# lucieDLE/TMRNet

Hardware: AMD Instinct MI355X
Metric: train frames/sec, TMRNet ResNet50 seq=10 LFB=40 (higher is better)
Workload: dtype fp32; 1 GPU; C2/C3: TMRNet ResNet50+LSTM+NLBlock train step; model=resnet_lstm (train_only_non-local_pretrained), global_batch=64, clips_per_gpu=64, seq_len=10, lfb_len=40, parallelism=dp1, input_transform=reference train transform (use_flip=1) on device

## Files before the change

### include/tmr.h

```cpp
#ifndef TMR_H_
#define TMR_H_

#ifdef TMR_HOST_ONLY
typedef struct ihipStream_t* hipStream_t;
#else
#include <hip/hip_runtime.h>
#endif
#include <stddef.h>
#include <stdint.h>

#ifdef __cplusplus
extern "C" {
#endif

#define TMR_ABI_VERSION 8

int tmr_abi_version(void);
const char* tmr_last_error(void);
void tmr_clear_error(void);

typedef struct tmr_conv_desc {
  int n, h, w, c;
  int k;
  int r, s, stride, pad;
// ... 347 lines not shown
                    void* ws, size_t ws_bytes, hipStream_t stream);


int tmr_linear_fwd(const float* x, int rows, int in, int out, const float* w, const float* bias,
                   float* y, hipStream_t stream);
int tmr_linear_bwd(const float* dy, const float* x, int rows, int in, int out, const float* w,
                   float* dx, float* dw, float* db, float beta, hipStream_t stream);

typedef struct tmr_nlblock_weights {
  const float *w1, *b1, *w2, *b2, *w3, *b3, *ln_w, *ln_b, *w4, *b4;
} tmr_nlblock_weights;
typedef struct tmr_nlblock_grads {
  float *w1, *b1, *w2, *b2, *w3, *b3, *ln_w, *ln_b, *w4, *b4;
} tmr_nlblock_grads;
size_t tmr_nlblock_saved_bytes(int b, int l);
size_t tmr_nlblock_ws_bytes(int b, int l);
int tmr_nlblock_fwd(const tmr_nlblock_weights* w, const float* st, const float* lt,
                    const int32_t* rows, int b, int l, const float* mask, float* out, void* saved,
                    size_t saved_bytes, void* ws, size_t ws_bytes, hipStream_t stream);
int tmr_nlblock_bwd(const tmr_nlblock_weights* w, const float* dout, const float* st,
                    const float* lt, const int32_t* rows, int b, int l, const float* mask,
                    const void* saved, size_t saved_bytes, float* dst, float* dlt,
                    const tmr_nlblock_grads* g, void* ws, size_t ws_bytes, hipStream_t stream);

size_t tmr_timeconv_saved_bytes(int b, int l);
size_t tmr_timeconv_ws_bytes(int b, int l);
int tmr_timeconv_fwd(const float* x, int b, int l, const float* w3, const float* b3,
                     const float* w5, const float* b5, const float* w7, const float* b7,
                     float* out, void* saved, size_t saved_bytes, void* ws, size_t ws_bytes,
                     hipStream_t stream);
int tmr_timeconv_wgrad(const float* dy, const float* x, int b, int l, const float* w3,
                       const float* w5, const float* w7, const void* saved, size_t saved_bytes,
                       float* dx, float* dw3, float* db3, float* dw5, float* db5, float* dw7,
                       float* db7, void* ws, size_t ws_bytes, hipStream_t stream);

size_t tmr_lstm_saved_bytes(int b, int t, int h);
size_t tmr_lstm_ws_bytes(int b, int t, int i, int h);
int tmr_lstm_fwd(const float* x, int b, int t, int i, int h, const float* w_ih,
                 const float* w_hh, const float* b_ih, const float* b_hh, float* y, float* hn,
                 float* cn, void* saved, size_t saved_bytes, void* ws, size_t ws_bytes,
                 hipStream_t stream);
int tmr_lstm_bwd(const float* dy, const float* x, int b, int t, int i, int h, const float* w_ih,
                 const float* w_hh, const float* y, const void* saved, size_t saved_bytes,
                 float* dx, float* dw_ih, float* dw_hh, float* db_ih, float* db_hh, void* ws,
                 size_t ws_bytes, hipStream_t stream);
size_t tmr_lstm_window_ws_bytes(int b, int t, int h);
int tmr_lstm_window_fwd(const float* gates, long nrows, const int32_t* rows, int b, int t, int h,
                        const float* w_hh, float* out, const int32_t* out_rows, void* ws,
                        size_t ws_bytes, hipStream_t stream);
int tmr_lstm_sync_status(const void* ws, unsigned* timeout_out, hipStream_t stream);
int tmr_lstm_status_or(const void* ws, int32_t* status, hipStream_t stream);
int tmr_test_hold_cus(int wgs, float ms, hipStream_t stream);
long tmr_dgrad_ws_launches(void);

int tmr_timeconv_max5_fwd(const float* x, const float* y1, const float* y2, const float* y3,
                          float* out, uint8_t* code, int b, int l, int c, hipStream_t stream);
int tmr_timeconv_max5_bwd(const float* dy, const uint8_t* code, float* d1, float* d2, float* d3,
                          float* dx, int b, int l, int c, hipStream_t stream);

int tmr_lstm_cell_fwd(const float* gx, int ldgx, const float* ghh, const float* c_prev,
                      float* h_out, int ldh, float* c_out, float* act, int b, int hdim,
                      hipStream_t stream);
int tmr_lstm_cell_bwd(const float* dh_out, int lddh, const float* dh_rec, const float* dc_next,
                      const float* act, const float* c, const float* c_prev, float* dgates,
                      int lddg, float* dc_prev, int b, int hdim, hipStream_t stream);

#ifdef __cplusplus
}
#endif
#endif
```

### tmrnet_amd/_lib.py

```python
import ctypes
import os

import torch

_HERE = os.path.dirname(os.path.abspath(__file__))
LIB_PATH = os.environ.get("TMR_LIB_PATH") or os.path.join(_HERE, "libtmr.so")

P = ctypes.c_void_p
I = ctypes.c_int
L = ctypes.c_long
F = ctypes.c_float
U64 = ctypes.c_uint64
SZ = ctypes.c_size_t


class ConvDesc(ctypes.Structure):
    _fields_ = [(n, ctypes.c_int) for n in
                ("n", "h", "w", "c", "k", "r", "s", "stride", "pad", "ho", "wo", "pad_w",
                 "x_ld", "y_ld", "math", "max_frames", "io", "groups")]


DP = ctypes.POINTER(ConvDesc)


# ... 100 lines not shown
    "tmr_splat_gap_bn": [P, P, P, P, I, I, I, I, P],
    "tmr_splat_att": [P, P, I, I, P],
    "tmr_splat_combine_bn": [P, P, P, P, P, I, I, I, I, P],
    "tmr_splat_bwd_reduce_bn": [P, P, P, P, P, P, P, P, I, I, I, I, P],
    "tmr_splat_bn0_coefs": [P, P, P, P, P, P, P, P, P, I, I, I, P],
    "tmr_splat_bwd_apply_bn": [P, P, P, P, P, P, P, P, P, I, I, I, I, P],
    "tmr_avgpool2d_fwd_a16": [P, P, I, I, I, I, I, I, I, I, I, I, P],
    "tmr_fill_f32": [P, L, F, P],
    "tmr_seq_last": [P, P, I, I, I, P],
    "tmr_seq_last_bwd": [P, P, P, I, I, I, P],
    "tmr_counters_add": [P, I, ctypes.c_int64, P],
    "tmr_center_cols": [P, I, I, P, P, P],
    "tmr_axpy": [I, F, P, P, P],
    "tmr_avgpool2d_fwd": [P, P, I, I, I, I, I, I, I, I, I, I, P],
    "tmr_avgpool2d_bwd": [P, P, I, I, I, I, I, I, I, I, I, I, P],
    "tmr_col_sum": [P, I, I, I, P, F, P],
    "tmr_dropout_mask": [P, L, F, U64, U64, P],
    "tmr_softmax_max": [P, I, I, P, P, P, P],
    "tmr_ce_sum": [P, P, P, I, I, F, P, P, P, P],
    "tmr_sgd_chunk": [],
    "tmr_sgd_step_multi": [P, I, ctypes.c_int64, P, P],
    "tmr_sgd_step": [P, P, P, L, F, F, F, F, I, I, P],
    "tmr_lfb_index": [P, I, P, I, I, P, P],
    "tmr_lfb_gather": [P, P, P, L, I, P],
    "tmr_layernorm_relu_fwd": [P, P, P, P, P, P, I, I, F, P],
    "tmr_layernorm_relu_bwd": [P, P, P, P, P, P, P, P, P, I, I, P],
    "tmr_residual_mask": [P, P, P, P, L, P],
    "tmr_mask_relu_fwd": [P, P, P, L, P],
    "tmr_mask_relu_bwd": [P, P, P, P, L, P],
    "tmr_mul": [P, P, P, P, L, P],
    "tmr_nl_attn_ws_bytes": [I, I, I],
    "tmr_nl_attn_fwd": [P, P, P, P, P, I, I, I, F, P, SZ, P],
    "tmr_nl_attn_bwd": [P, P, P, P, P, P, P, I, I, I, F, P, SZ, P],
    "tmr_linear_fwd": [P, I, I, I, P, P, P, P],
    "tmr_linear_bwd": [P, P, I, I, I, P, P, P, P, F, P],
    "tmr_nlblock_saved_bytes": [I, I],
    "tmr_nlblock_ws_bytes": [I, I],
    "tmr_nlblock_fwd": [P, P, P, P, I, I, P, P, P, SZ, P, SZ, P],
    "tmr_nlblock_bwd": [P, P, P, P, P, I, I, P, P, SZ, P, P, P, P, SZ, P],
    "tmr_timeconv_saved_bytes": [I, I],
    "tmr_timeconv_ws_bytes": [I, I],
    "tmr_timeconv_fwd": [P, I, I, P, P, P, P, P, P, P, P, SZ, P, SZ, P],
    "tmr_timeconv_wgrad": [P, P, I, I, P, P, P, P, SZ, P, P, P, P, P, P, P, P, SZ, P],
    "tmr_lstm_saved_bytes": [I, I, I],
    "tmr_lstm_ws_bytes": [I, I, I, I],
    "tmr_lstm_fwd": [P, I, I, I, I, P, P, P, P, P, P, P, P, SZ, P, SZ, P],
    "tmr_lstm_bwd": [P, P, I, I, I, I, P, P, P, P, SZ, P, P, P, P, P, P, SZ, P],
    "tmr_lstm_window_ws_bytes": [I, I, I],
    "tmr_lstm_window_fwd": [P, L, P, I, I, I, P, P, P, P, SZ, P],
    "tmr_lstm_sync_status": [P,ctypes.POINTER(ctypes.c_uint), P],
    "tmr_lstm_status_or": [P, P, P],
    "tmr_test_hold_cus": [I, F, P],
    "tmr_dgrad_ws_launches": [],
    "tmr_timeconv_max5_fwd": [P, P, P, P, P, P, I, I, I, P],
    "tmr_timeconv_max5_bwd": [P, P, P, P, P, P, I, I, I, P],
    "tmr_lstm_cell_fwd": [P, I, P, P, P, I, P, P, I, I, P],
    "tmr_lstm_cell_bwd": [P, I, P, P, P, P, P, P, I, P, I, I, P],
}
_RESTYPES = {
    "tmr_last_error": ctypes.c_char_p,
    "tmr_clear_error": None,
    "tmr_conv2d_wgrad_ws_bytes": SZ,
    "tmr_dgrad_ws_launches": L,
    "tmr_resize_tmp_bytes": SZ,
    "tmr_margin_ws_bytes": SZ,
    "tmr_jpeg_ws_bytes": SZ,
    "tmr_bn_ws_bytes": SZ,
    "tmr_bn_parts_ws_bytes": SZ,
    "tmr_bn_bwd_parts_ds_ws_bytes": SZ,
    "tmr_sgd_chunk": ctypes.c_int64,
    "tmr_nl_attn_ws_bytes": SZ,
    "tmr_nlblock_saved_bytes": SZ,
    "tmr_nlblock_ws_bytes": SZ,
    "tmr_timeconv_saved_bytes": SZ,
    "tmr_timeconv_ws_bytes": SZ,
    "tmr_lstm_saved_bytes": SZ,
    "tmr_lstm_ws_bytes": SZ,
    "tmr_lstm_window_ws_bytes": SZ,
}

_lib = None


def lib():
    global _lib
    if _lib is None:
        if not os.path.exists(LIB_PATH):
            raise RuntimeError(
                "libtmr.so not found at %s: build it with `make` or "
                "`python -c 'import __graft_entry__ as g; g.build()'` (no CPU fallback exists)"
                % LIB_PATH)
        h = ctypes.CDLL(LIB_PATH)
        for name, args in SIGNATURES.items():
            fn = getattr(h, name)
            fn.argtypes = args
            fn.restype = _RESTYPES.get(name, ctypes.c_int)
        _lib = h
    return _lib


def exported_symbols():
    return list(SIGNATURES)


def _conv(a):
    if isinstance(a, torch.Tensor):
        return ctypes.c_void_p(a.data_ptr())
    return a


def stream_ptr(device=None):
    return ctypes.c_void_p(torch.cuda.current_stream(device).cuda_stream)


def call(name, *args):
    fn = getattr(lib(), name)
# ... 16 lines not shown
```

### tmrnet_amd/csrc/gemm16_kernel.h

```cpp
#pragma once
#include "gemm16_select.h"
#include <cstring>
#include <type_traits>

namespace tmrg {

typedef short s16x4_t __attribute__((ext_vector_type(4)));
typedef short s16x8_t __attribute__((ext_vector_type(8)));
#define TMR_LDS_AS __attribute__((address_space(3)))

__device__ __forceinline__ void glds16(__amdgpu_buffer_rsrc_t r, unsigned char* dst, uint32_t voff) {
  __builtin_amdgcn_raw_ptr_buffer_load_lds(r, (TMR_LDS_AS void*)dst, 16, voff, 0, 0, 0);
}

template <int R>
__device__ __forceinline__ int mn_swz(int k) {
  return R >= 128 ? ((k & 3) << 2) : (((k >> 1) & 1) << 2);
}

__device__ __forceinline__ void store_g8(const GemmArgs& a, long off, const float (&v)[8]) {
  if (a.g16) {
    uint32_t w[4];
#pragma unroll
    for (int e = 0; e < 4; ++e)
// ... 793 lines not shown
  const int ch = w / PAR_G, off = w - ch * PAR_G;
  int base = 0, prev = 0;
  cls = 0;
  t = 1 << 30;
  for (int n = p.n; n > 0; --n) {
    const int tn = (p.c[n - 1].tiles + PAR_G - 1) / PAR_G;
    const int span = n * (tn - prev);
    if (ch < base + span) {
      const int q = ch - base;
      cls = q % n;
      t = (prev + q / n) * PAR_G + off;
      return;
    }
    base += span;
    prev = tn;
  }
}

template <int BM, int BN, int WM, int WN, int F32, int EPF = 0>
__global__ __launch_bounds__(64 * WM * WN, (occ16<BM, BN, WM, WN, 2>()))
void gemm16_par_kernel(const GemmPar p) {
  int w, split;
  xcd_work(w, split);
  int cls, t;
  par_tile(p, w, cls, t);
  cls = __builtin_amdgcn_readfirstlane(cls);
  t = __builtin_amdgcn_readfirstlane(t);
  if (t >= p.c[cls].tiles) return;
  GemmArgs a = p.a;
  const ParClass& c = p.c[cls];
  auto own = [](auto v) {
    asm volatile("" : "+s"(v));
    return v;
  };
  a.M = own(c.M);
  a.K = own(c.K);
  a.ntaps = own(c.ntaps);
  a.tapS = own(c.tapS);
  a.tapSinv = own(c.tapSinv);
  a.oy0 = own(c.oy0);
  a.ox0 = own(c.ox0);
  a.wr0 = own(c.wr0);
  a.ws0 = own(c.ws0);
  a.oyc = own(c.oyc);
  a.oxc = own(c.oxc);
  a.dHW = FastDiv{own(c.dHW.d), own(c.dHW.m), own(c.dHW.s)};
  a.dW = FastDiv{own(c.dW.d), own(c.dW.m), own(c.dW.s)};
  a.bn_part = own(c.bn_part);
  gemm16_body<MODE_DGRAD, BM, BN, WM, WN, 0, 1, F32, 2, EPF>(a, t, 0);
}

}
#include "gemm16_ws.h"
namespace tmrg {

template <int MODE, int BM, int BN, int WM, int WN, int F32>
int launch16_cfg(const GemmArgs& a, bool tapv, dim3 grid, hipStream_t st) {
  const dim3 blk(64 * WM * WN);
  if constexpr (MODE == MODE_FWD && F32 == 0) {
    if (a.c16 && a.scale) return launch16_inf16<BM, BN, WM, WN>(a, tapv, grid, st);
  }
  constexpr int kmax = 64;
  if constexpr (MODE == MODE_FWD && F32 == 0 && WM * WN == 4 &&
                ((BM == 128 && BN == 128) || (BM == 256 && BN == 64))) {
    if (!tapv && a.K > 0 && a.K <= kmax) {
      hipLaunchKernelGGL((gemm16_kernel<MODE, BM, BN, WM, WN, 0, 1, F32, 1>), grid, blk, 0, st, a);
      TMR_CHECK_LAUNCH("gemm16_kernel (one stage)");
      return 0;
    }
  }
  if constexpr (MODE == MODE_FWD && F32 == 0 && BM == 256 && BN == 256) {
    if (!tapv && a.K > 0 && a.K <= kmax) {
      const dim3 g2((unsigned)(cdiv(a.M, 256) * cdiv(a.N, 128)), grid.y, 1);
      hipLaunchKernelGGL((gemm16_kernel<MODE, 256, 128, 4, 2, 0, 1, F32, 1>), g2, dim3(512), 0, st, a);
      TMR_CHECK_LAUNCH("gemm16_kernel (one stage, 256x128)");
      return 0;
    }
  }
  constexpr bool FORMS = MODE == MODE_DGRAD && TMR_EPI_FORMS &&
                         (WM * WN == 4 || (WM * WN == 8 && TMR_EPI_LATE_F > 0));
  if constexpr (FORMS) {
    const int f = a.bn_part != nullptr ? epi_form(a) : 0;
    if (f == (F32 ? 2 : 1)) {
      if (tapv)
        hipLaunchKernelGGL((gemm16_kernel<MODE, BM, BN, WM, WN, 1, 1, F32, 2, F32 ? 2 : 1>), grid, blk, 0, st, a);
      else
        hipLaunchKernelGGL((gemm16_kernel<MODE, BM, BN, WM, WN, 0, 1, F32, 2, F32 ? 2 : 1>), grid, blk, 0, st, a);
      TMR_CHECK_LAUNCH("gemm16_kernel (dgrad epilogue form)");
      return 0;
    }
  }
  if (tapv) {
    hipLaunchKernelGGL((gemm16_kernel<MODE, BM, BN, WM, WN, 1, 1, F32>), grid, blk, 0, st, a);
  } else {
    hipLaunchKernelGGL((gemm16_kernel<MODE, BM, BN, WM, WN, 0, 1, F32>), grid, blk, 0, st, a);
  }
  TMR_CHECK_LAUNCH(F32 ? "gemm16_kernel (fp32)" : "gemm16_kernel");
  return 0;
}

template <int MODE, int F32>
int launch16_switch(const GemmArgs& a, int cfg, bool tapv, dim3 grid, hipStream_t st) {
  switch (cfg) {
    case 1: return launch16_cfg<MODE, 256, 128, 4, 2, F32>(a, tapv, grid, st);
    case 2: return launch16_cfg<MODE, 128, 128, 2, 2, F32>(a, tapv, grid, st);
    case 3: return launch16_cfg<MODE, 256, 64, 4, 1, F32>(a, tapv, grid, st);
    case 4: return launch16_cfg<MODE, 64, 256, 1, 4, F32>(a, tapv, grid, st);
    case 7: return launch16_cfg<MODE, 128, 128, 4, 2, F32>(a, tapv, grid, st);
    case 5: return launch16_cfg<MODE, 64, 64, 2, 2, F32>(a, tapv, grid, st);
    case 0: return launch16_cfg<MODE, 256, 256, 2, 4, F32>(a, tapv, grid, st);
    case 6: return launch16_cfg<MODE, 256, 256, 4, 4, F32>(a, tapv, grid, st);
    default: break;
  }
  TMR_CHECK_ARG(false, "gemm16: no tile config %d", cfg);
  return 1;
}

template <int MODE, int F32>
int check16(const GemmArgs& a, int cfg) {
  TMR_CHECK_ARG(((uintptr_t)a.A & 15) == 0 && ((uintptr_t)a.B & 15) == 0,
                "gemm (LDS-DMA path): operands must be 16-B aligned");
  constexpr bool f32 = F32 != 0;
  TMR_CHECK_ARG((a.prec == TMR_MATH_F32) == f32, "gemm (LDS-DMA path): precision dispatch");
  TMR_CHECK_ARG(!f32 || (a.lds % 4 == 0 && a.log2C >= 2 &&
                         (MODE == MODE_DGRAD ? (a.ldbt % 4 == 0 && a.N % 8 == 0 && a.ldc % 4 == 0 &&
                                                ((uintptr_t)a.C & 15) == 0)
                                             : a.ldb % 4 == 0)),
                "gemm (fp32 LDS-DMA path): 4-channel pieces, 16-B row strides (view %d)", MODE);
  const Cfg16 c = kCfgs16[cfg];
  TMR_CHECK_ARG(a.bn_part == nullptr || a.bn_mask != 3 ||
                    (MODE == MODE_DGRAD && !(c.bm == 256 && c.bn == 256)),
                "gemm: ReLU-mask bits (mask 3) need the LDS-DMA dgrad's LDS-staged epilogue (tile %dx%d)",
                c.bm, c.bn);
  TMR_CHECK_ARG(!a.g16 || (MODE == MODE_DGRAD && a.bn_part != nullptr &&
                           !(c.bm == 256 && c.bn == 256) && ((uintptr_t)a.C & 15) == 0 &&
                           a.ldc % 8 == 0),
                "gemm: a bf16 BN-backward gradient (TMR_IO_G16) needs the fused LDS-staged dgrad "
                "epilogue, 16-B aligned rows (tile %dx%d)", c.bm, c.bn);
  TMR_CHECK_ARG((!a.Cold && !a.cold16) ||
                    (MODE == MODE_DGRAD && a.bn_part != nullptr && !(c.bm == 256 && c.bn == 256) &&
                     ((uintptr_t)(a.Cold ? a.Cold : a.C) & 15) == 0),
                "gemm: a separate / bf16 old dx needs the fused LDS-staged dgrad epilogue (tile %dx%d)",
                c.bm, c.bn);
  return 0;
}

template <int MODE, int F32>
int launch_gemm16_t(const GemmArgs& a, int splits, hipStream_t st) {
  constexpr bool f32 = F32 != 0;
  const int cfg = pick_cfg16(a.M, a.N, a.K, MODE, f32);
  const Cfg16 c = kCfgs16[cfg];
  if (const int rc = check16<MODE, F32>(a, cfg)) return rc;
  dim3 grid(cdiv(a.M, c.bm) * cdiv(a.N, c.bn), splits, 1);
  if (grid.x == 0) return 0;
  const int bk = f32 ? 32 : 64;
  const bool tapv = MODE != MODE_WGRAD && a.ntaps > 1 && ((1 << a.log2C) % bk) != 0;
  if (MODE == MODE_WGRAD && (c.bm < 64 || c.bn < 64)) return -1;
  if constexpr (MODE == MODE_DGRAD) {
    const int rc = launch_dgrad_ws<F32>(a, cfg, st);
    if (rc >= 0) return rc;
  }
  return launch16_switch<MODE, F32>(a, cfg, tapv, grid, st);
}

template <int MODE, int F32>
int launch_gemm16(const GemmArgs& a, int splits, hipStream_t st) {
  return launch_gemm16_t<MODE, F32>(a, splits, st);
}

template <int F32>
int launch_gemm16_par(const GemmArgs* as, int n, hipStream_t st) {
  constexpr bool f32 = F32 != 0;
  static_assert(sizeof(GemmPar) <= 4096, "kernel argument size");
  if (n < 2 || n > PAR_MAX) return -1;
  const int cfg = pick_cfg16(as[0].M, as[0].N, as[0].K, MODE_DGRAD, f32);
  const int bk = f32 ? 32 : 64;
  for (int i = 0; i < n; ++i) {
    const GemmArgs& a = as[i];
    if ((a.prec == TMR_MATH_F32) != f32 || !use16(a, MODE_DGRAD)) return -1;
    if (pick_cfg16(a.M, a.N, a.K, MODE_DGRAD, f32) != cfg) return -1;
    if (a.ntaps > 1 && ((1 << a.log2C) % bk) != 0) return -1;
  }
  switch (cfg) {
    case 1: case 2: case 3: case 5: case 7: break;
    default: return -1;
  }
  GemmPar p{};
  p.n = n;

  const Cfg16 c = kCfgs16[cfg];
  auto own = [](const GemmArgs& a, int tiles) {
    return ParClass{a.M, a.K, a.ntaps, a.tapS, a.tapSinv, a.oy0, a.ox0, a.wr0, a.ws0, a.oyc, a.oxc,
                    tiles, a.dHW, a.dW, a.bn_part};
  };
  auto put = [](GemmArgs& a, const ParClass& q) {
    a.M = q.M; a.K = q.K; a.ntaps = q.ntaps; a.tapS = q.tapS; a.tapSinv = q.tapSinv;
    a.oy0 = q.oy0; a.ox0 = q.ox0; a.wr0 = q.wr0; a.ws0 = q.ws0; a.oyc = q.oyc; a.oxc = q.oxc;
    a.dHW = q.dHW; a.dW = q.dW; a.bn_part = q.bn_part;
  };
  int ord[PAR_MAX];
  for (int i = 0; i < n; ++i) ord[i] = i;
  auto tiles = [&](const GemmArgs& a) { return (int)(cdiv(a.M, c.bm) * cdiv(a.N, c.bn)); };
  for (int i = 1; i < n; ++i)
// ... 39 lines not shown
```

### tmrnet_amd/csrc/gemm16_select.h

```cpp
#pragma once
#include "gemm_kernel.h"

namespace tmrg {

struct Cfg16 { int bm, bn; };
constexpr Cfg16 kCfgs16[] = {{256, 256}, {256, 128}, {128, 128}, {256, 64}, {64, 256}, {64, 64},
                              {256, 256},
                              {128, 128}};

inline bool use32(const GemmArgs& a, int mode) {
  if (a.prec != TMR_MATH_F32 || a.sab) return false;
  if (mode == MODE_DGRAD) return a.wt != 0;
  if (!a.dma32) return false;
  if ((((uintptr_t)a.A | (uintptr_t)a.B) & 15) != 0) return false;
  if (mode == MODE_WGRAD)
    return a.M % 4 == 0 && a.log2C >= 2 && a.ldb % 4 == 0 && a.lds % 4 == 0 && a.N % 4 == 0;
  return a.lds % 4 == 0 && a.ldb % 4 == 0 && a.log2C >= 2 && (a.ntaps != 1 || a.K % 4 == 0);
}

inline bool use16(const GemmArgs& a, int mode) {
  if (a.prec == TMR_MATH_F32) return use32(a, mode);
  if (a.prec != TMR_MATH_BF16 || a.sab != 3) return false;
  if (mode == MODE_DGRAD && !a.wt) return false;
  if (a.lds % 8) return false;
  if (mode == MODE_WGRAD) return a.M % 8 == 0 && a.log2C >= 3 && a.ldb % 8 == 0 && a.N % 8 == 0;
  if (mode == MODE_FWD && a.ldb % 8) return false;
  if (mode == MODE_DGRAD && a.ldbt % 8) return false;
  return a.ntaps == 1 ? (a.K % 8 == 0 && (mode == MODE_FWD || a.log2C >= 3)) : a.log2C >= 3;
}

inline long cfg16_tiles(long M, long N, int c) {
  return ((M + kCfgs16[c].bm - 1) / kCfgs16[c].bm) * ((N + kCfgs16[c].bn - 1) / kCfgs16[c].bn);
}

inline int pick_cfg16(long M, long N, long K, int mode, bool f32 = false) {
  static const int forced = env_int("TMR_GEMM16_CFG", -1);
  if (forced >= 0 && forced < (int)(sizeof(kCfgs16) / sizeof(kCfgs16[0]))) return forced;
  int cfg;
  if (f32 && mode == MODE_WGRAD) {
    if (M <= 64) return (N <= 64 || N >= 512) ? 5 : 4;
    if (N <= 64) return 5;
    if (M >= 256 && N >= 256 && 2.0 * M * N * K >= 100e9) return 6;
    return 7;
  }
  if (f32 && M >= 256 && mode == MODE_DGRAD && N >= 512) {
    static const int wide = env_int("TMR_DGRAD32_WIDE_CFG", 7);
    return cfg16_tiles(M, N, wide) >= 256 ? wide : 2;
  }
  if (f32 && M >= 256 && mode == MODE_FWD && N == 128)
    return cfg16_tiles(M, N, 7) >= 256 ? 7 : 2;
  if (mode == MODE_WGRAD) {
    if (M <= 64) cfg = N <= 64 ? 5 : (N >= 512 ? 4 : 2);
    else if (N <= 64) cfg = 3;
    else cfg = (M >= 256 && N >= 1024 && K * cfg16_tiles(M, N, 6) >= (1L << 21)) ? 6 : 7;
  } else if (N <= 64) {
    cfg = M >= 256 ? 3 : 5;
  } else if (mode == MODE_FWD && N >= 256 && M >= 256) {
    cfg = 6;
  } else {
    cfg = 2;
  }
  if (mode != MODE_WGRAD && cfg16_tiles(M, N, cfg) < (f32 && cfg == 6 ? 224 : 256)) {
    for (const int c2 : {1, 2, 5}) {
      if ((long)kCfgs16[c2].bm * kCfgs16[c2].bn >= (long)kCfgs16[cfg].bm * kCfgs16[cfg].bn ||
          cfg16_tiles(M, N, c2) <= cfg16_tiles(M, N, cfg))
        continue;
      cfg = c2;
      if (cfg16_tiles(M, N, cfg) >= 256) break;
    }
  }
  return cfg;
}

inline int gemm_tile_bm(const GemmArgs& a, int mode) {
  return use16(a, mode) ? kCfgs16[pick_cfg16(a.M, a.N, a.K, mode, a.prec == TMR_MATH_F32)].bm
                        : kCfgs[pick_cfg(a.M, a.N, a.K, mode)].bm;
}
inline long gemm_tiles(const GemmArgs& a, int mode) {
  return use16(a, mode) ? cfg16_tiles(a.M, a.N, pick_cfg16(a.M, a.N, a.K, mode, a.prec == TMR_MATH_F32))
                        : cfg_tiles(a.M, a.N, pick_cfg(a.M, a.N, a.K, mode));
}

constexpr int PAR_MAX = 4;
struct ParClass {
  int M, K, ntaps, tapS, tapSinv, oy0, ox0, wr0, ws0, oyc, oxc, tiles;
  FastDiv dHW, dW;
  float2* bn_part;
};
struct GemmPar {
  GemmArgs a;
  ParClass c[PAR_MAX];
  int n;
};
constexpr int PAR_G = 64;

extern long g_dgrad_ws_launches;

template <int F32>
int launch_gemm16_par(const GemmArgs* as, int n, hipStream_t st);
extern template int launch_gemm16_par<0>(const GemmArgs*, int, hipStream_t);
extern template int launch_gemm16_par<1>(const GemmArgs*, int, hipStream_t);
template <int MODE, int F32>
int launch_gemm16(const GemmArgs& a, int splits, hipStream_t st);
extern template int launch_gemm16<MODE_FWD, 0>(const GemmArgs&, int, hipStream_t);
extern template int launch_gemm16<MODE_FWD, 1>(const GemmArgs&, int, hipStream_t);
extern template int launch_gemm16<MODE_DGRAD, 0>(const GemmArgs&, int, hipStream_t);
extern template int launch_gemm16<MODE_DGRAD, 1>(const GemmArgs&, int, hipStream_t);
extern template int launch_gemm16<MODE_WGRAD, 0>(const GemmArgs&, int, hipStream_t);
extern template int launch_gemm16<MODE_WGRAD, 1>(const GemmArgs&, int, hipStream_t);

template <int BM, int BN, int WM, int WN>
int launch16_inf16(const GemmArgs& a, bool tapv, dim3 grid, hipStream_t st);
extern template int launch16_inf16<256, 128, 4, 2>(const GemmArgs&, bool, dim3, hipStream_t);
extern template int launch16_inf16<128, 128, 2, 2>(const GemmArgs&, bool, dim3, hipStream_t);
extern template int launch16_inf16<256, 64, 4, 1>(const GemmArgs&, bool, dim3, hipStream_t);
extern template int launch16_inf16<64, 256, 1, 4>(const GemmArgs&, bool, dim3, hipStream_t);
extern template int launch16_inf16<128, 128, 4, 2>(const GemmArgs&, bool, dim3, hipStream_t);
extern template int launch16_inf16<64, 64, 2, 2>(const GemmArgs&, bool, dim3, hipStream_t);
extern template int launch16_inf16<256, 256, 2, 4>(const GemmArgs&, bool, dim3, hipStream_t);
extern template int launch16_inf16<256, 256, 4, 4>(const GemmArgs&, bool, dim3, hipStream_t);

}
```

### tmrnet_amd/csrc/gemm_conv.hip

```cpp
#include "gemm16_select.h"

#include <type_traits>

using namespace tmrg;

namespace {

__device__ __forceinline__ float split_sum(const float* __restrict__ slabs, int nsplit, long slab,
                                           long src) {
  float s = 0.f;
  int p = 0;
  for (; p + 8 <= nsplit; p += 8) {
    float v[8];
#pragma unroll
    for (int u = 0; u < 8; ++u) v[u] = slabs[(p + u) * slab + src];
#pragma unroll
    for (int u = 0; u < 8; ++u) s += v[u];
  }
  for (; p < nsplit; ++p) s += slabs[p * slab + src];
  return s;
}

__global__ void wgrad_reduce_kernel(const float* __restrict__ slabs, int nsplit, long slab,
                                    float* __restrict__ out, int Cout, int ntaps, int Cpad,
// ... 63 lines not shown
}

static uint32_t clamp_bytes(long elems) {
  long b = elems * 4;
  return b >= 0x80000000L ? 0x80000000u : (uint32_t)b;
}

int ilog2_exact(int v) {
  if (v <= 0 || (v & (v - 1))) return -1;
  int l = 0;
  while ((1 << l) < v) ++l;
  return l;
}

bool aligned16(const void* p) { return (((uintptr_t)p) & 15) == 0; }

void set_taps(GemmArgs& a, int nR, int nS) {
  a.ntaps = nR * nS;
  a.tapS = nS > 0 ? nS : 1;
  a.tapSinv = (65536 + a.tapS - 1) / a.tapS;
}

void set_grid(GemmArgs& a, int n, int hg, int wg) {
  (void)n;
  a.dHW = make_fastdiv((uint32_t)(hg * wg));
  a.dW = make_fastdiv((uint32_t)wg);
}

}

static int conv_fwd_args(const tmr_conv_desc* d, const float* x, const float* w_krsc,
                         const float* bias, float* y, float beta, GemmArgs& a, bool& al) {
  TMR_CHECK_ARG(d, "tmr_conv2d_fwd: null descriptor");
  TMR_CHECK_ARG(d->math == TMR_MATH_F32 || d->math == TMR_MATH_BF16, "tmr_conv2d: bad math mode %d", d->math);
  TMR_CHECK_ARG((d->io & ~(TMR_IO_ENGINE | TMR_IO_CLASSES | TMR_IO_TILES)) == 0 || d->math == TMR_MATH_BF16, "tmr_conv2d: bf16-stored operands (io %d) need TMR_MATH_BF16", d->io);
  const int lc = ilog2_exact(d->c);
  TMR_CHECK_ARG(lc >= 2, "tmr_conv2d_fwd: stored input channels %d must be a power of two >= 4", d->c);
  a = GemmArgs{};
  a.A = x; a.B = w_krsc; a.C = y; a.bias = bias;
  a.M = d->n * d->ho * d->wo; a.N = d->k; a.K = d->r * d->s * d->c;
  a.log2C = lc;
  set_taps(a, d->r, d->s);
  a.oy0 = -d->pad; a.ox0 = -d->pad_w; a.dyr = 1; a.dxs = 1;
  set_grid(a, d->n, d->ho, d->wo);
  a.Hs = d->h; a.Ws = d->w; a.sy = d->stride; a.sx = d->stride;
  a.lds = xld_of(d); a.ldb = a.K; a.ldc = yld_of(d); a.beta = beta;
  a.Abytes = clamp_bytes_e(span((long)d->n * d->h * d->w, a.lds, d->c), esz_x(d));
  a.prec = d->math;
  a.Bbytes = clamp_bytes_e((long)d->k * a.K, esz_w(d));
  a.sab = ((d->io & TMR_IO_X_BF16) ? 1 : 0) | ((d->io & TMR_IO_W_BF16) ? 2 : 0);
  a.Cbytes = clamp_bytes(span((long)d->n * d->ho * d->wo, a.ldc, d->k));
  a.c16 = (d->io & TMR_IO_Y_BF16) ? 2 : 0;
  a.dma32 = d->math == TMR_MATH_F32;
  al = aligned16(x) && aligned16(w_krsc) && (d->k % 4 == 0) && (a.lds % 4 == 0);
  return 0;
}

static int frames_per_launch(const tmr_conv_desc* d) {
  const long xf = (long)d->h * d->w * xld_of(d) * 4;
  const long yf = (long)d->ho * d->wo * yld_of(d) * 4;
  const long mx = xf > yf ? xf : yf;
  long f = mx > 0 ? 0x7fffffffL / mx : d->n;
  if (d->max_frames > 0 && d->max_frames < f) f = d->max_frames;
  if (f > d->n) f = d->n;
  return (int)(f > 0 ? f : 1);
}

static tmr_conv_desc chunk_desc(const tmr_conv_desc* d, int nc) {
  tmr_conv_desc c = *d;
  c.n = nc;
  return c;
}

static int stats_parts_of(const tmr_conv_desc* d) {
  GemmArgs a;
  bool al;
  if (conv_fwd_args(d, nullptr, nullptr, nullptr, nullptr, 0.f, a, al)) return 0;
  return cdiv(a.M, gemm_tile_bm(a, MODE_FWD));
}

static long x_frame(const tmr_conv_desc* d) { return (long)d->h * d->w * xld_of(d); }
static long y_frame(const tmr_conv_desc* d) { return (long)d->ho * d->wo * yld_of(d); }

static int ngroups(const tmr_conv_desc* d) { return d->groups > 1 ? d->groups : 1; }
static int group_split(const tmr_conv_desc* d, tmr_conv_desc& g) {
  const int G = ngroups(d);
  TMR_CHECK_ARG(d->c % G == 0 && d->k % G == 0, "tmr_conv2d: channels %d / %d not divisible by %d groups",
                d->c, d->k, G);
  g = *d;
  g.x_ld = xld_of(d);
  g.y_ld = yld_of(d);
  g.c = d->c / G;
  g.k = d->k / G;
  g.groups = 0;
  return 0;
}
static long group_wsize(const tmr_conv_desc* g) { return (long)g->k * g->r * g->s * g->c; }

TMR_API int tmr_conv2d_fwd(const tmr_conv_desc* d, const float* x, const float* w_krsc,
                           const float* bias, float* y, float beta, hipStream_t stream) {
  TMR_CHECK_ARG(d, "tmr_conv2d_fwd: null descriptor");
  if (ngroups(d) > 1) {
    tmr_conv_desc g;
    if (group_split(d, g)) return 1;
    for (int i = 0; i < d->groups; ++i) {
      const int rc = tmr_conv2d_fwd(&g, adv(x, (long)i * g.c, esz_x(d)), adv(w_krsc, i * group_wsize(&g), esz_w(d)),
// ... 294 lines not shown
        a.Cold = fz->old;
        a.cold16 = fz->old16;
        a.io_tiles = (d->io & TMR_IO_TILES) ? 1 : 0;
        fz->part += nmt * fz->part_ld;
        fz->nparts += nmt;
      }
      bool al = aligned16(dy) && aligned16(w_krsc) && aligned16(dx) && a.lds % 4 == 0;
      if (par) {
        pend[npend] = a;
        pend_al[npend++] = al;
        continue;
      }
      const int rc = launch_gemm<MODE_DGRAD>(a, al, 1, stream);
      if (rc) return rc;
    }
  }
  if (npend > 0) {
    int rc = launch_gemm_dgrad_par(pend, npend, stream);
    if (rc < 0) {
      rc = 0;
      for (int i = 0; i < npend && rc == 0; ++i)
        rc = launch_gemm<MODE_DGRAD>(pend[i], pend_al[i], 1, stream);
    }
    if (rc) return rc;
  }
  return 0;
}

static int dgrad_bnbwd_run(const tmr_conv_desc* d, const float* dy, const float* w_krsc, float* dx,
                           float beta, BnBwdFuse* fz, hipStream_t stream) {
  const int fc = frames_per_launch(d);
  const long px_frame = (long)d->h * d->w * xld_of(d);
  float2* part0 = fz->part;
  for (int f0 = 0; f0 < d->n; f0 += fc) {
    const tmr_conv_desc c = chunk_desc(d, d->n - f0 < fc ? d->n - f0 : fc);
    BnBwdFuse fc_ = *fz;
    fc_.y = adv(fz->y, f0 * px_frame, esz_bn(d));
    fc_.z = fz->mask == 3 ? (const float*)((const uint32_t*)fz->z + f0 * px_frame / 32)
                          : adv(fz->z, f0 * px_frame, esz_bn(d));
    fc_.nparts = 0;
    if (fz->old) fc_.old = adv(fz->old, f0 * x_frame(d), fz->old16 ? 2 : 4);
    int rc = conv_dgrad_impl(&c, adv(dy, f0 * y_frame(d), esz_dy(d)), w_krsc,
                             dx ? adv(dx, f0 * x_frame(d), esz_dx(d)) : nullptr, beta, stream, &fc_);
    if (rc) return rc;
    fz->part = fc_.part;
    fz->nparts += fc_.nparts;
  }
  fz->part = part0;
  return 0;
}

long tmrg::g_dgrad_ws_launches = 0;
TMR_API long tmr_dgrad_ws_launches(void) { return __atomic_load_n(&g_dgrad_ws_launches, __ATOMIC_RELAXED); }

TMR_API int tmr_conv2d_dgrad_bnbwd_parts(const tmr_conv_desc* d) {
  if (!d || d->n <= 0) {
    tmr_set_error("tmr_conv2d_dgrad_bnbwd_parts: null or empty descriptor");
    return -1;
  }
  if (d3_dgrad(d)) return tmr_d3_dgrad_parts(d->n, d->h, d->w, d->c, d->k);
  tmr_conv_desc g = *d;
  if (ngroups(d) > 1 && group_split(d, g)) return -1;
  BnBwdFuse fz{};
  fz.count_only = true;
  fz.part_ld = g.c;
  if (dgrad_bnbwd_run(&g, nullptr, nullptr, nullptr, 1.f, &fz, nullptr)) return -1;
  return (int)fz.nparts;
}

static int dgrad_bnbwd_entry(const tmr_conv_desc* d, const float* dy, const float* w_krsc,
                             float* dx, float beta, const void* dx_old, int old_bf16,
                             const float* y, const float* z, const float* scale,
                             const float* shift, const float* mean, int mask, void* parts,
                             size_t parts_bytes, hipStream_t stream);

TMR_API int tmr_conv2d_dgrad_bnbwd(const tmr_conv_desc* d, const float* dy, const float* w_krsc,
                                   float* dx, float beta, const float* y, const float* z,
                                   const float* scale, const float* shift, const float* mean,
                                   int mask, void* parts, size_t parts_bytes, hipStream_t stream) {
  TMR_CHECK_ARG(d, "tmr_conv2d_dgrad_bnbwd: null descriptor");
  return dgrad_bnbwd_entry(d, dy, w_krsc, dx, beta, nullptr, (d->io & TMR_IO_G16) ? 1 : 0, y, z,
                           scale, shift, mean, mask, parts, parts_bytes, stream);
}

TMR_API int tmr_conv2d_dgrad_bnbwd_acc(const tmr_conv_desc* d, const float* dy,
                                       const float* w_krsc, void* dx, float beta,
                                       const void* dx_old, int old_bf16, const float* y,
                                       const float* z, const float* scale, const float* shift,
                                       const float* mean, int mask, void* parts,
                                       size_t parts_bytes, hipStream_t stream) {
  TMR_CHECK_ARG(d, "tmr_conv2d_dgrad_bnbwd_acc: null descriptor");
  TMR_CHECK_ARG(beta != 0.f && dx_old && ((uintptr_t)dx_old & 15) == 0 &&
                    (d->io & TMR_IO_G16) && (d->io & TMR_IO_WT_BF16),
                "tmr_conv2d_dgrad_bnbwd_acc: needs beta != 0, a 16-B aligned old dx and a bf16 "
                "output (TMR_IO_G16) on the bf16 LDS-DMA engine (TMR_IO_WT_BF16)");
  return dgrad_bnbwd_entry(d, dy, w_krsc, (float*)dx, beta, dx_old, old_bf16 ? 1 : 0, y, z, scale,
                           shift, mean, mask, parts, parts_bytes, stream);
}

static int dgrad_bnbwd_entry(const tmr_conv_desc* d, const float* dy, const float* w_krsc,
                             float* dx, float beta, const void* dx_old, int old_bf16,
                             const float* y, const float* z, const float* scale,
                             const float* shift, const float* mean, int mask, void* parts,
                             size_t parts_bytes, hipStream_t stream) {
  TMR_CHECK_ARG(xld_of(d) == d->c, "tmr_conv2d_dgrad_bnbwd: dx must be dense (x_ld == c)");
  TMR_CHECK_ARG(ngroups(d) == 1 || mask != 3,
// ... 301 lines not shown
```

### tmrnet_amd/ops.py

```python
import contextlib
import threading
import weakref

import numpy as np
import torch

from ._lib import call, query, stream_ptr, ConvDesc
from . import health
import ctypes

f32 = torch.float32

PROF = None


class _prof:
    def __init__(self, kind, flops, shape=None, nbytes=0):
        self.kind, self.flops, self.shape, self.nbytes = kind, flops, shape, nbytes

    def __enter__(self):
        if PROF is not None:
            self.e0 = torch.cuda.Event(enable_timing=True)
            self.e1 = torch.cuda.Event(enable_timing=True)
            self.e0.record()
# ... 33 lines not shown
MATH = {"fp32": 0, "bf16": 1}
_SUFFIX = {"fp32": "", "bf16": "_bf16"}
MAX_FRAMES = 0


IO_X, IO_W, IO_DY, IO_WT = 1, 2, 4, 8
IO_Y, IO_BN = 16, 32
IO_WT32 = 64
IO_G16 = 128
IO_ENGINE = 256
IO_CLASSES = 512
IO_TILES = 1024

_ENGINE = [False]


@contextlib.contextmanager
def engine_only():
    prev = _ENGINE[0]
    _ENGINE[0] = True
    try:
        yield
    finally:
        _ENGINE[0] = prev


def engine_forced():
    return _ENGINE[0]


_CLASSES = [False]


@contextlib.contextmanager
def dgrad_class_launches():
    prev = _CLASSES[0]
    _CLASSES[0] = True
    try:
        yield
    finally:
        _CLASSES[0] = prev

_TILES = [False]


@contextlib.contextmanager
def dgrad_tile_launches():
    prev = _TILES[0]
    _TILES[0] = True
    try:
        yield
    finally:
        _TILES[0] = prev


BF16 = torch.bfloat16


def _io(x=None, w=None, dy=None, wt=False):
    if wt and w.dtype == f32:
        if (dy is not None and dy.dtype != f32) or (x is not None and x.dtype != f32):
            raise RuntimeError("fp32 transposed (CRSK) weights need fp32 operands")
        return IO_WT32
    io = 0
    for t, bit in ((x, IO_X), (w, IO_WT if wt else IO_W), (dy, IO_DY)):
        if t is not None and t.dtype == torch.bfloat16:
            io |= bit
    if wt and not io & IO_WT:
        raise RuntimeError("transposed (CRSK) weights must be bf16 or fp32")
    return io


def _dgrad_w(w, wt, groups=1):
    if wt and groups > 1:
        g, cg, r, s, kg = w.shape
        return kg * g, r, s, cg * g
    if wt:
        c, r, s, k = w.shape
    else:
        k, r, s, c = w.shape
        c *= groups
    return k, r, s, c


def _esz(t):
    return t.element_size() if t is not None else 4


def conv_desc(n, h, w, c, k, r, s, stride, pad, pad_w=None, x_ld=0, y_ld=0, math="fp32", io=0,
              groups=1):
    pad_w = pad if pad_w is None else pad_w
    ho = (h + 2 * pad - r) // stride + 1
    wo = (w + 2 * pad_w - s) // stride + 1
    if io and io != IO_WT32 and math != "bf16":
        raise RuntimeError("bf16-stored conv operands need math='bf16'")
    if io & IO_WT32 and math != "fp32":
        raise RuntimeError("fp32 transposed weights (TMR_IO_WT_F32) need math='fp32'")
    if engine_forced():
        io |= IO_ENGINE
    if _CLASSES[0] and stride == 2:
        io |= IO_CLASSES
    if _TILES[0] and r == 1 and s == 1 and stride == 1:
        io |= IO_TILES
    return ConvDesc(n, h, w, c, k, r, s, stride, pad, ho, wo, pad_w, x_ld, y_ld, MATH[math],
                    MAX_FRAMES, io, groups if groups > 1 else 0)

# ... 1040 lines not shown
```

Measured before the change: 3799 frames/s.

## Add persistent N-walk fp32 forward GEMM kernel with overlapped stores and BN stats

```diff
diff --git a/include/tmr.h b/include/tmr.h
--- a/include/tmr.h
+++ b/include/tmr.h
@@ -423,6 +423,7 @@
 int tmr_lstm_status_or(const void* ws, int32_t* status, hipStream_t stream);
 int tmr_test_hold_cus(int wgs, float ms, hipStream_t stream);
 long tmr_dgrad_ws_launches(void);
+long tmr_fwd_walk_launches(void);
 
 int tmr_timeconv_max5_fwd(const float* x, const float* y1, const float* y2, const float* y3,
                           float* out, uint8_t* code, int b, int l, int c, hipStream_t stream);
diff --git a/tmrnet_amd/_lib.py b/tmrnet_amd/_lib.py
--- a/tmrnet_amd/_lib.py
+++ b/tmrnet_amd/_lib.py
@@ -176,6 +176,7 @@
     "tmr_lstm_status_or": [P, P, P],
     "tmr_test_hold_cus": [I, F, P],
     "tmr_dgrad_ws_launches": [],
+    "tmr_fwd_walk_launches": [],
     "tmr_timeconv_max5_fwd": [P, P, P, P, P, P, I, I, I, P],
     "tmr_timeconv_max5_bwd": [P, P, P, P, P, P, I, I, I, P],
     "tmr_lstm_cell_fwd": [P, I, P, P, P, I, P, P, I, I, P],
@@ -186,6 +187,7 @@
     "tmr_clear_error": None,
     "tmr_conv2d_wgrad_ws_bytes": SZ,
     "tmr_dgrad_ws_launches": L,
+    "tmr_fwd_walk_launches": L,
     "tmr_resize_tmp_bytes": SZ,
     "tmr_margin_ws_bytes": SZ,
     "tmr_jpeg_ws_bytes": SZ,
diff --git a/tmrnet_amd/csrc/gemm16_kernel.h b/tmrnet_amd/csrc/gemm16_kernel.h
--- a/tmrnet_amd/csrc/gemm16_kernel.h
+++ b/tmrnet_amd/csrc/gemm16_kernel.h
@@ -869,6 +869,7 @@
 
 }
 #include "gemm16_ws.h"
+#include "gemm16_nwalk.h"
 namespace tmrg {
 
 template <int MODE, int BM, int BN, int WM, int WN, int F32>
@@ -892,6 +893,12 @@
       hipLaunchKernelGGL((gemm16_kernel<MODE, 256, 128, 4, 2, 0, 1, F32, 1>), g2, dim3(512), 0, st, a);
       TMR_CHECK_LAUNCH("gemm16_kernel (one stage, 256x128)");
       return 0;
+    }
+  }
+  if constexpr (MODE == MODE_FWD && F32 == 1 && BM == 256 && BN == 256 && WM == 4 && WN == 4) {
+    if (!tapv) {
+      const int rc = launch_fwd_walk(a, st);
+      if (rc >= 0) return rc;
     }
   }
   constexpr bool FORMS = MODE == MODE_DGRAD && TMR_EPI_FORMS &&
@@ -965,7 +972,8 @@
 template <int MODE, int F32>
 int launch_gemm16_t(const GemmArgs& a, int splits, hipStream_t st) {
   constexpr bool f32 = F32 != 0;
-  const int cfg = pick_cfg16(a.M, a.N, a.K, MODE, f32);
+  int cfg = pick_cfg16(a.M, a.N, a.K, MODE, f32);
+  if (MODE == MODE_FWD && f32 && a.stats != nullptr && fwd_walk_shape(a)) cfg = 6;
   const Cfg16 c = kCfgs16[cfg];
   if (const int rc = check16<MODE, F32>(a, cfg)) return rc;
   dim3 grid(cdiv(a.M, c.bm) * cdiv(a.N, c.bn), splits, 1);
diff --git a/tmrnet_amd/csrc/gemm16_nwalk.h b/tmrnet_amd/csrc/gemm16_nwalk.h
--- /dev/null
+++ b/tmrnet_amd/csrc/gemm16_nwalk.h
@@ -0,0 +1,292 @@
+#pragma once
+#include <utility>
+
+namespace tmrg {
+
+#ifndef TMR_NWALK_EXP
+#define TMR_NWALK_EXP 0
+#endif
+#ifndef TMR_NWALK_SPREAD
+#define TMR_NWALK_SPREAD 1
+#endif
+template <int V>
+using ic = std::integral_constant<int, V>;
+
+template <class F, int... C>
+__device__ __forceinline__ void nwalk_chunks(F&& f, std::integer_sequence<int, C...>) {
+  (f(std::integral_constant<int, C>{}), ...);
+}
+
+template <int NCH, int EXACT>
+__global__ __launch_bounds__(1024, 4) void gemm16_kernel_nwalk(const GemmArgs a, const int run) {
+  constexpr int BM = 256, BN = 128, NW = 16, WN = 4, TM = 2;
+  constexpr uint32_t ES = 4u;
+  constexpr int EPC = 4, BK = 32;
+  constexpr int ABYTES = BM * 128, BBYTES = BN * 128, STAGE = ABYTES + BBYTES;
+  constexpr int NIA = ABYTES / (1024 * NW), NIB = BBYTES / (1024 * NW);
+  static_assert(NIA == 2 && NIB == 1, "LDS-DMA pieces per wave");
+  static_assert(NCH == 0 || NCH == 2 || NCH == 4, "store chunks (whole quarters)");
+  constexpr int SPK = NCH > 0 ? 32 / NCH : 32;
+  constexpr int RED = 4 * BN * 4;
+  __shared__ __attribute__((aligned(1024))) unsigned char smem[2 * STAGE + RED];
+  float* const red = reinterpret_cast<float*>(smem + 2 * STAGE);
+
+  const int tid = threadIdx.x;
+  const int lane = tid & 63;
+  const int wave = __builtin_amdgcn_readfirstlane(tid >> 6);
+  const int wm = wave / WN, wn = wave % WN;
+  const int l31 = lane & 31, hh = lane >> 5;
+
+  const int nst = a.N / BN;
+  const int total = ((a.M + BM - 1) / BM) * nst;
+  int bid, split;
+  xcd_work(bid, split);
+  const int g0 = bid * run;
+  const int nj = min(run, total - g0);
+  int mi = g0 / nst, ns = g0 - mi * nst;
+  int mi_n = mi, ns_n = ns;
+  auto advance = [&]() {
+    mi = mi_n;
+    ns = ns_n;
+    ns_n = ns + 1 == nst ? 0 : ns + 1;
+    mi_n = ns + 1 == nst ? mi + 1 : mi;
+  };
+  advance();
+  const int nk = (NCH > 0 && EXACT) ? NCH : (a.K + BK - 1) / BK;
+  const int rep = NCH > 0 ? nk / NCH : 0;
+
+  const __amdgpu_buffer_rsrc_t rA = make_rsrc(a.A, a.Abytes);
+  const __amdgpu_buffer_rsrc_t rB = make_rsrc(a.B, a.Bbytes);
+  const __amdgpu_buffer_rsrc_t rC = make_rsrc(a.C, a.Cbytes);
+  const uint32_t sbytes =
+      (uint32_t)(((long)((a.M + BM - 1) / BM - 1) * a.part_ld + a.N) * (long)sizeof(float4));
+  const __amdgpu_buffer_rsrc_t rS = make_rsrc(reinterpret_cast<const float*>(a.stats), sbytes);
+
+  int arow[NIA], ach[NIA];
+#pragma unroll
+  for (int q = 0; q < NIA; ++q) {
+    arow[q] = 8 * (wave + NW * q) + (lane >> 3);
+    ach[q] = EPC * ((lane & 7) ^ ((arow[q] >> 1) & 7));
+  }
+  const int brow = 8 * wave + (lane >> 3);
+  const int bch = EPC * ((lane & 7) ^ ((brow >> 1) & 7));
+  auto stage = [&](int sm, int sn, int kt, int buf, bool live) {
+    const int kb = kt * BK;
+    unsigned char* As = smem + buf * STAGE;
+    unsigned char* Bs = As + ABYTES;
+#pragma unroll
+    for (int q = 0; q < NIA; ++q) {
+      const int m = sm * BM + arow[q];
+      const bool ok = live && m < a.M && kb + ach[q] < a.K;
+      const uint32_t off = (uint32_t)m * (uint32_t)a.lds * ES + (uint32_t)(kb + ach[q]) * ES;
+      glds16(rA, As + 1024 * (wave + NW * q), ok ? off : OOB);
+    }
+    const bool okb = live && kb + bch < a.K;
+    const uint32_t boff =
+        (uint32_t)(sn * BN + brow) * (uint32_t)a.ldb * ES + (uint32_t)(kb + bch) * ES;
+    glds16(rB, Bs + 1024 * wave, okb ? boff : OOB);
+  };
+  auto stage_next = [&](int jj, int kt, int buf) {
+    const bool last = kt + 1 == nk;
+    stage(last ? mi_n : mi, last ? ns_n : ns, last ? 0 : kt + 1, buf, !last || jj + 1 < nj);
+  };
+
+  const int kx = (l31 >> 1) & 7;
+  const int arow0 = wm * (BM / 4) + l31;
+  const int brow0 = wn * (BN / WN) + l31;
+  auto frags = [&](int buf, int s, f32x4_t (&av)[TM], f32x4_t& bv) {
+    const unsigned char* As = smem + buf * STAGE;
+    const unsigned char* Bs = As + ABYTES;
+    const int ch = (2 * s + hh) ^ kx;
+#pragma unroll
+    for (int i = 0; i < TM; ++i)
+      av[i] = *reinterpret_cast<const f32x4_t*>(As + (arow0 + 32 * i) * 128 + (ch << 4));
+    bv = *reinterpret_cast<const f32x4_t*>(Bs + brow0 * 128 + (ch << 4));
+  };
+  floatx16 acc[TM], prev[TM];
+#pragma unroll
+  for (int i = 0; i < TM; ++i)
+#pragma unroll
+    for (int r = 0; r < 16; ++r) {
+      acc[i][r] = 0.f;
+      prev[i][r] = 0.f;
+    }
+  auto mfmas = [&](const f32x4_t (&av)[TM], const f32x4_t& bv) {
+    if constexpr (TMR_NWALK_EXP == 2) {
+      asm volatile("" ::"v"(av[0]), "v"(av[1]), "v"(bv));
+      return;
+    }
+    __builtin_amdgcn_s_setprio(1);
+#pragma unroll
+    for (int t = 0; t < 4; ++t)
+#pragma unroll
+      for (int i = 0; i < TM; ++i)
+        acc[i] = __builtin_amdgcn_mfma_f32_32x32x2f32(av[i][t], bv[t], acc[i], 0, 0, 0);
+    __builtin_amdgcn_s_setprio(0);
+  };
+
+  const int wrel0 = wm * (BM / 4) + 4 * hh;
+  int prow0 = a.M;
+  uint32_t pbase = 0u, poff = OOB;
+  float pmean = 0.f, pm2 = 0.f, pnrows = 0.f;
+  const uint32_t ldc4 = (uint32_t)a.ldc * 4u;
+  auto store_regs = [&](auto e0c, auto nc) {
+    constexpr int e0 = decltype(e0c)::value, n = decltype(nc)::value;
+    if constexpr (TMR_NWALK_EXP == 1) return;
+#pragma unroll
+    for (int e = e0; e < e0 + n; ++e) {
+      const int i = e >> 4, r = e & 15;
+      const int rel = 32 * i + (r & 3) + 8 * (r >> 2);
+      const bool ok = prow0 + rel < a.M;
+      const float v = prev[i][r] + 0.f;
+      __builtin_amdgcn_raw_buffer_store_b32(__builtin_bit_cast(uint32_t, v), rC,
+                                            ok ? pbase + (uint32_t)rel * ldc4 : OOB, 0, 0);
+    }
+  };
+  auto store_stats = [&]() {
+    const u32x4_t q = {__float_as_uint(pnrows), __float_as_uint(pmean), __float_as_uint(pm2), 0u};
+    __builtin_amdgcn_raw_buffer_store_b128(q, rS, poff, 0, 0);
+    poff = OOB;
+  };
+  auto ktile = [&](int jj, int kt, int buf, auto waitc, auto&& stores) {
+    constexpr int WAITC = decltype(waitc)::value;
+    asm volatile("s_waitcnt vmcnt(%0)" ::"n"(WAITC) : "memory");
+    ws_barrier();
+    f32x4_t a0[TM], a1[TM], b0, b1;
+    frags(buf, 0, a0, b0);
+    stage_next(jj, kt, buf ^ 1);
+    if constexpr (!TMR_NWALK_SPREAD) {
+      stores(ic<0>{}); stores(ic<1>{}); stores(ic<2>{}); stores(ic<3>{});
+    }
+    frags(buf, 1, a1, b1);
+    if constexpr (TMR_NWALK_SPREAD) stores(ic<0>{});
+    mfmas(a0, b0);
+    frags(buf, 2, a0, b0);
+    if constexpr (TMR_NWALK_SPREAD) stores(ic<1>{});
+    mfmas(a1, b1);
+    frags(buf, 3, a1, b1);
+    if constexpr (TMR_NWALK_SPREAD) stores(ic<2>{});
+    mfmas(a0, b0);
+    if constexpr (TMR_NWALK_SPREAD) stores(ic<3>{});
+    mfmas(a1, b1);
+  };
+  auto finish = [&]() {
+    const int m0 = mi * BM, n0 = ns * BN;
+    const int wrow0 = m0 + wrel0;
+    const float fnrows = (float)min(BM, a.M - m0);
+    auto valid = [&](int i, int r) { return wrow0 + 32 * i + (r & 3) + 8 * (r >> 2) < a.M; };
+    const int rc = wm * BN + wn * (BN / WN) + l31, cc = wn * (BN / WN) + l31;
+    float t = 0.f;
+#pragma unroll
+    for (int i = 0; i < TM; ++i)
+#pragma unroll
+      for (int r = 0; r < 16; ++r) t += valid(i, r) ? acc[i][r] + 0.f : 0.f;
+    t += __shfl_xor(t, 32, 64);
+    if (hh == 0) red[rc] = t;
+    ws_barrier();
+    float mj = 0.f;
+#pragma unroll
+    for (int w = 0; w < 4; ++w) mj += red[w * BN + cc];
+    mj = mj / fnrows;
+    ws_barrier();
+    t = 0.f;
+#pragma unroll
+    for (int i = 0; i < TM; ++i)
+#pragma unroll
+      for (int r = 0; r < 16; ++r) {
+        const float d = acc[i][r] + 0.f - mj;
+        t += valid(i, r) ? d * d : 0.f;
+      }
+    t += __shfl_xor(t, 32, 64);
+    if (hh == 0) red[rc] = t;
+    ws_barrier();
+    float m2 = 0.f;
+#pragma unroll
+    for (int w = 0; w < 4; ++w) m2 += red[w * BN + cc];
+    pmean = mj;
+    pm2 = m2;
+    pnrows = fnrows;
+    poff = (wm == 0 && hh == 0)
+               ? (uint32_t)((long)mi * a.part_ld + n0 + cc) * (uint32_t)sizeof(float4)
+               : OOB;
+    prow0 = wrow0;
+    pbase = (uint32_t)wrow0 * ldc4 + (uint32_t)(n0 + cc) * 4u;
+#pragma unroll
+    for (int i = 0; i < TM; ++i)
+#pragma unroll
+      for (int r = 0; r < 16; ++r) {
+        prev[i][r] = acc[i][r];
+        acc[i][r] = 0.f;
+      }
+    advance();
+  };
+  using std::integral_constant;
+  constexpr integral_constant<int, 0> c0{};
+  constexpr integral_constant<int, 32> c32{};
+
+  stage(mi, ns, 0, 0, true);
+  if constexpr (NCH > 0) {
+    asm volatile("s_waitcnt vmcnt(0)" ::: "memory");
+    for (int jj = 0; jj < nj; ++jj) {
+      auto chunk = [&](auto cc) {
+        constexpr int c = decltype(cc)::value;
+        constexpr int W = EXACT ? (c == 1 ? SPK + 1 : SPK) : 0;
+        const int kt0 = EXACT ? c : c * rep;
+        ktile(jj, kt0, kt0 & 1, integral_constant<int, W>{}, [&](auto pc) {
+          constexpr int p = decltype(pc)::value;
+          store_regs(ic<c * SPK + p * (SPK / 4)>{}, ic<SPK / 4>{});
+          if constexpr (c == 0 && p == 0) store_stats();
+        });
+        if constexpr (!EXACT)
+          for (int u = 1; u < rep; ++u) ktile(jj, kt0 + u, (kt0 + u) & 1, c0, [](auto) {});
+      };
+      nwalk_chunks(chunk, std::make_integer_sequence<int, NCH>{});
+      finish();
+    }
+  } else {
+    int g = 0;
+    for (int jj = 0; jj < nj; ++jj) {
+      for (int kt = 0; kt < nk; ++kt) {
+        ktile(jj, kt, g & 1, c0, [&](auto pc) {
+          constexpr int p = decltype(pc)::value;
+          if (kt == 0) {
+            store_regs(ic<8 * p>{}, ic<8>{});
+            if constexpr (p == 0) store_stats();
+          }
+        });
+        ++g;
+      }
+      finish();
+    }
+  }
+  store_regs(c0, c32);
+  store_stats();
+}
+
+inline int launch_fwd_walk(const GemmArgs& a, hipStream_t st) {
+  static const int run_env = env_int("TMR_FWD_WALK_RUN", 0);
+  static const int rounds_env = env_int("TMR_FWD_WALK_ROUNDS", 2);
+  const int rounds = rounds_env > 0 ? rounds_env : 2;
+  if (a.io_tiles || a.stats == nullptr || !fwd_walk_shape(a)) return -1;
+  if (a.bias || a.scale || a.res || a.relu || a.beta != 0.f) return -1;
+  const long total = cdiv(a.M, 256) * (long)(a.N / 128);
+  long run = cdiv(total, 256L * rounds);
+  if (run < 2) run = 2;
+  if (run_env > 0) run = run_env;
+  const long nwg = cdiv(total, run);
+  TMR_CHECK_ARG(nwg < (1L << 31), "gemm (N-walk forward): %ld workgroups", nwg);
+  const dim3 grid((unsigned)nwg), blk(1024);
+  auto go = [&](auto kern) {
+    hipLaunchKernelGGL(kern, grid, blk, 0, st, a, (int)run);
+    TMR_CHECK_LAUNCH("gemm16_kernel_nwalk");
+    __atomic_fetch_add(&g_fwd_walk_launches, 1L, __ATOMIC_RELAXED);
+    return 0;
+  };
+  const int nk = cdiv(a.K, 32);
+  if (nk == 2) return go(gemm16_kernel_nwalk<2, 1>);
+  if (nk == 4) return go(gemm16_kernel_nwalk<4, 1>);
+  if (nk % 2 == 0) return go(gemm16_kernel_nwalk<2, 0>);
+  return go(gemm16_kernel_nwalk<0, 0>);
+}
+
+}
diff --git a/tmrnet_amd/csrc/gemm16_select.h b/tmrnet_amd/csrc/gemm16_select.h
--- a/tmrnet_amd/csrc/gemm16_select.h
+++ b/tmrnet_amd/csrc/gemm16_select.h
@@ -72,7 +72,24 @@
   return cfg;
 }
 
+#ifndef TMR_FWD_WALK
+#define TMR_FWD_WALK 1
+#endif
+#ifndef TMR_FWD_WALK_KMAX
+#define TMR_FWD_WALK_KMAX 256
+#endif
+inline bool fwd_walk_shape(const GemmArgs& a) {
+  static const int on = env_int("TMR_FWD_WALK", TMR_FWD_WALK);
+  static const int kmax = env_int("TMR_FWD_WALK_KMAX", TMR_FWD_WALK_KMAX);
+  if (!on || !use32(a, MODE_FWD) || a.c16) return false;
+  if (a.ntaps != 1 || a.sy != 1 || a.sx != 1 || a.oy0 != 0 || a.ox0 != 0 ||
+      (long)a.Hs * a.Ws != (long)a.dHW.d || a.Ws != (int)a.dW.d)
+    return false;
+  return a.M >= 256 && a.N >= 256 && a.N % 128 == 0 && a.K > 0 && a.K % 8 == 0 && a.K <= kmax;
+}
+
 inline int gemm_tile_bm(const GemmArgs& a, int mode) {
+  if (mode == MODE_FWD && fwd_walk_shape(a)) return 256;
   return use16(a, mode) ? kCfgs16[pick_cfg16(a.M, a.N, a.K, mode, a.prec == TMR_MATH_F32)].bm
                         : kCfgs[pick_cfg(a.M, a.N, a.K, mode)].bm;
 }
@@ -95,6 +112,7 @@
 constexpr int PAR_G = 64;
 
 extern long g_dgrad_ws_launches;
+extern long g_fwd_walk_launches;
 
 template <int F32>
 int launch_gemm16_par(const GemmArgs* as, int n, hipStream_t st);
diff --git a/tmrnet_amd/csrc/gemm_conv.hip b/tmrnet_amd/csrc/gemm_conv.hip
--- a/tmrnet_amd/csrc/gemm_conv.hip
+++ b/tmrnet_amd/csrc/gemm_conv.hip
@@ -139,6 +139,7 @@
   a.Cbytes = clamp_bytes(span((long)d->n * d->ho * d->wo, a.ldc, d->k));
   a.c16 = (d->io & TMR_IO_Y_BF16) ? 2 : 0;
   a.dma32 = d->math == TMR_MATH_F32;
+  a.io_tiles = (d->io & TMR_IO_TILES) ? 1 : 0;
   al = aligned16(x) && aligned16(w_krsc) && (d->k % 4 == 0) && (a.lds % 4 == 0);
   return 0;
 }
@@ -539,6 +540,8 @@
 
 long tmrg::g_dgrad_ws_launches = 0;
 TMR_API long tmr_dgrad_ws_launches(void) { return __atomic_load_n(&g_dgrad_ws_launches, __ATOMIC_RELAXED); }
+long tmrg::g_fwd_walk_launches = 0;
+TMR_API long tmr_fwd_walk_launches(void) { return __atomic_load_n(&g_fwd_walk_launches, __ATOMIC_RELAXED); }
 
 TMR_API int tmr_conv2d_dgrad_bnbwd_parts(const tmr_conv_desc* d) {
   if (!d || d->n <= 0) {
diff --git a/tmrnet_amd/ops.py b/tmrnet_amd/ops.py
--- a/tmrnet_amd/ops.py
+++ b/tmrnet_amd/ops.py
@@ -109,6 +109,10 @@
         yield
     finally:
         _TILES[0] = prev
+
+
+def fwd_tile_launches():
+    return dgrad_tile_launches()
 
 
 BF16 = torch.bfloat16
```

After: 3810 frames/s, median of 6. About the same (+0.3%).
